# bennyguo/instant-nsr-pl

Measured on NVIDIA H100. Metric: rays/sec fwd+bwd (NeRF-Synthetic lego shape), higher is better.
Workload: dtype f16

## Files before the change

instant-nsr-pl_b200/csrc/nerf_fused_bwd.cu:

```cuda
#include <stdlib.h>
#include "nerf_fused.cuh"
#include "wgmma.cuh"

namespace {

constexpr int kWarps = 4;
constexpr int kThreads = kWarps * 32;
constexpr int kRows = kWarps * 16;
constexpr int kCtasPerSm = 2;

constexpr int T_X0 = 0;
constexpr int T_H1 = T_X0 + kRows * NF_LD32;
constexpr int T_CI = T_H1 + kRows * NSR_LD64;
constexpr int T_G1 = T_CI + kRows * NF_LD32;
constexpr int T_G2 = T_G1 + kRows * NSR_LD64;
constexpr int T_DC3 = T_G2 + kRows * NSR_LD64;
constexpr int T_DG2 = T_DC3 + kRows * 24;
constexpr int T_DG1 = T_DG2 + kRows * NSR_LD64;
constexpr int T_DO = T_DG1 + kRows * NSR_LD64;
constexpr int T_DH1 = T_DO + kRows * 24;
constexpr int T_X0B = T_DH1 + kRows * NSR_LD64;
constexpr int T_TOTAL = T_X0B + kRows * NF_LD32;
constexpr int S_XYZ = 0, S_DS = S_XYZ + kRows * 6, S_DRGB = S_DS + kRows, S_ROWF = S_DRGB + kRows * 3;
constexpr size_t kSmemBytes = (size_t)(NF_W_TOTAL + T_TOTAL) * sizeof(__half) + 2 * S_ROWF * sizeof(float);
// ... 499 lines not shown
            }
          }
        }
        a_dc3[0][0][0] = nsr_pack_h2(dp[0], dp[1]);
        a_dc3[0][0][1] = nsr_pack_h2(dp[2], dp[3]);
        a_dc3[0][0][2] = 0u;
        a_dc3[0][0][3] = 0u;
        canon_store_afrag<1>(a_dc3, slot + SL_DC3, 16, r0);
      }
      uint32_t a_d[1][4][4];
      nsr_zero_acc(acc);
      nsr_gemm_wt<1, 1, 8>(acc, a_dc3, W + NF_OFF_CW3, NSR_LD64);
      relu_mask_pack(acc, a_g2, a_d);
      canon_store_afrag<4>(a_d, slot + SL_DG2, 64, r0);
      nsr_zero_acc(acc);
      nsr_gemm_wt<1, 4, 8>(acc, a_d, W + NF_OFF_CW2, NSR_LD64);
      relu_mask_pack(acc, a_g1, a_d);
      canon_store_afrag<4>(a_d, slot + SL_DG1, 64, r0);
      nsr_zero_acc(acc16);
      nsr_gemm_wt<1, 4, 2>(acc16, a_d, W + NF_OFF_CW1, NF_LD32);
      if (c == 0) {
        if (ia < n) acc16[0][0][0] += dsr[0] * loss_scale;
        if (ib < n) acc16[0][0][2] += dsr[1] * loss_scale;
      }
      uint32_t a_do[1][1][4];
      nsr_acc_to_afrag<1, 2>(acc16, a_do, NSR_ACT_NONE);
      canon_store_afrag<1>(a_do, slot + SL_DO, 16, r0);
      nsr_zero_acc(acc);
      nsr_gemm_wt<1, 1, 8>(acc, a_do, W + NF_OFF_DW2, NSR_LD64);
      relu_mask_pack(acc, a_h1, a_d);
      canon_store_afrag<4>(a_d, slot + SL_DH1, 64, r0);
      nsr_proxy_fence();
      mbar_arrive(full_bar(s));
      float accE[1][4][4];
      nsr_zero_acc(accE);
      nsr_gemm_wt<1, 4, 4>(accE, a_d, W + NF_OFF_DW1, NF_LD32);
#pragma unroll
      for (int hh = 0; hh < 2; ++hh) {
        const int64_t i = hh ? ib : ia;
        if (i < n) {
#pragma unroll
          for (int nt = 0; nt < 4; ++nt) denc_out[i * 16 + nt * 4 + c] = nsr_pack_h2(accE[0][nt][hh * 2], accE[0][nt][hh * 2 + 1]);
        }
      }
    }
  } else {
    float w_dw1[16], w_dw2t[8], w_cw1[16], w_cw2[32], w_cw3t[8];
#pragma unroll
    for (int i = 0; i < 32; ++i) {
      if (i < 8) w_dw2t[i] = w_cw3t[i] = 0.f;
      if (i < 16) w_dw1[i] = w_cw1[i] = 0.f;
      w_cw2[i] = 0.f;
    }
    for (int64_t it = 0; it < my_tiles; ++it) {
      const int s = (int)(it % kNetSlots);
      mbar_wait(full_bar(s), (uint32_t)((it / kNetSlots) & 1), nullptr, 0);
      const uint32_t sl = sbase + N_SLOTS + (uint32_t)s * kSlotBytes;
      nsr_wg_fence();
#pragma unroll
      for (int kk = 0; kk < 4; ++kk) {
        nsr_wgmma_n32<1, 1>(w_dw1, nsr_wg_desc_mn(sl + SL_DH1, 64, kk), nsr_wg_desc_mn(sl + SL_X0, 32, kk), 1u);
        nsr_wgmma_n16<1, 1>(w_dw2t, nsr_wg_desc_mn(sl + SL_H1, 64, kk), nsr_wg_desc_mn(sl + SL_DO, 16, kk), 1u);
        nsr_wgmma_n32<1, 1>(w_cw1, nsr_wg_desc_mn(sl + SL_DG1, 64, kk), nsr_wg_desc_mn(sl + SL_CI, 32, kk), 1u);
        nsr_wgmma_n64<1, 1>(w_cw2, nsr_wg_desc_mn(sl + SL_DG2, 64, kk), nsr_wg_desc_mn(sl + SL_G1, 64, kk), 1u);
        nsr_wgmma_n16<1, 1>(w_cw3t, nsr_wg_desc_mn(sl + SL_G2, 64, kk), nsr_wg_desc_mn(sl + SL_DC3, 16, kk), 1u);
      }
      nsr_wg_commit();
      nsr_wg_wait0();
      nsr_wg_fence_regs(w_dw1);
      nsr_wg_fence_regs(w_dw2t);
      nsr_wg_fence_regs(w_cw1);
      nsr_wg_fence_regs(w_cw2);
      nsr_wg_fence_regs(w_cw3t);
      mbar_arrive(empty_bar(s));
    }
    if (my_tiles > 0) {
      net_flush(w_dw1, grad_dparams, 32, 1, inv_scale);
      net_flush(w_dw2t, grad_dparams + 64 * 32, 1, 64, inv_scale);
      net_flush(w_cw1, grad_cparams, 32, 1, inv_scale);
      net_flush(w_cw2, grad_cparams + 64 * 32, 64, 1, inv_scale);
      net_flush(w_cw3t, grad_cparams + 64 * 32 + 64 * 64, 1, 64, inv_scale);
    }
  }
}

}

namespace {

constexpr int kMergeLevels = 8;

template <int MINB>
__global__ void __launch_bounds__(256, MINB) nerf_table_scatter_kernel(const __grid_constant__ nsr_grid_t g, const float* __restrict__ xyz, int stride,
                                                                 const __half2* __restrict__ denc, float loss_scale,
                                                                 const float* __restrict__ amax_ptr, float* __restrict__ grad_table,
                                                                 int64_t n_cap, const int64_t* __restrict__ n_dev, int l_begin, int l_end) {
  const int64_t n = n_dev ? min(*n_dev, n_cap) : n_cap;
  if (loss_scale <= 0.f) {
    const float amax = fmaxf(__ldg(amax_ptr), 1e-30f);
    loss_scale = exp2f(fminf(fmaxf(floorf(log2f(256.f / amax)), -24.f), 60.f));
  }
  const float inv_scale = 1.f / loss_scale;
  const int lane = threadIdx.x & 31;
  const int64_t n32 = (n + 31) & ~31ll;
  for (int64_t i = blockIdx.x * 256ll + threadIdx.x; i < n32; i += (int64_t)gridDim.x * 256) {
    const bool ok = i < n;
    float x = 0.f, y = 0.f, z = 0.f;
    if (ok) {
      x = xyz[i * stride];
      y = xyz[i * stride + 1];
      z = xyz[i * stride + 2];
    }
    uint2 dq = make_uint2(0u, 0u);
#pragma unroll 1
    for (int l = l_begin; l < l_end; ++l) {
      float2 d = make_float2(0.f, 0.f);
      if (ok) {
        if (l == l_begin || (l & 1) == 0) dq = __ldg(reinterpret_cast<const uint2*>(denc + i * 16 + (l & ~1)));
        const uint32_t h = (l & 1) ? dq.y : dq.x;
        d = __half22float2(*reinterpret_cast<const __half2*>(&h));
        d.x *= inv_scale;
        d.y *= inv_scale;
      }
      const LevelInfo li = nsr_level(g, l);
      uint32_t cx, cy, cz, idx[8];
      float fx, fy, fz;
      nsr_pos_fract(x, li.scale, cx, fx);
      nsr_pos_fract(y, li.scale, cy, fy);
// ... 165 lines not shown
```

instant-nsr-pl_b200/fused.py:

```python
import ctypes
import math

import torch

from . import ops
from .lib import lib, ptr, stream, check_cuda, contig, NerfT
from .nerfacc import ContractionType

SCATTER_LEVEL_GROUPS = ((12, 16), (8, 12), (0, 8))


class _NerfRender(torch.autograd.Function):

    @staticmethod
    def forward(ctx, dparams, cparams, fused, rays, jitter):
        st = fused.trace(rays, jitter)
        n_rays, cap = rays.shape[0], st['cap']
        dev = rays.device
        acc_rgb = torch.zeros(n_rays, 3, device=dev)
        opacity = torch.zeros(n_rays, 1, device=dev)
        depth = torch.zeros(n_rays, 1, device=dev)
        sig = torch.empty(cap, device=dev)
        rgbs = torch.empty(cap, 3, device=dev)
        weights = torch.empty(cap, device=dev)
        need_grad = dparams.requires_grad or cparams.requires_grad
        enc = torch.empty(cap, 32, dtype=torch.float16, device=dev) if need_grad else None
        dh, ch = fused.dparams_half(), fused.cparams_half()
        k_dev = st['offsets_k'][n_rays:]
        lib.call('nsr_nerf_render_fwd', fused.ref(), ptr(rays), ptr(st['ri']), ptr(st['ts']), ptr(st['te']), ptr(st['trans']), ptr(dh),
                 ptr(ch), ptr(enc), ptr(sig), ptr(rgbs), ptr(weights), ptr(acc_rgb), ptr(opacity), ptr(depth), cap, ptr(k_dev), stream())
        ctx.fused, ctx.n_rays, ctx.cap = fused, n_rays, cap
        ctx.set_materialize_grads(False)
        ctx.save_for_backward(rays, st['ri'], st['ts'], st['te'], st['trans'], st['offsets_k'], enc, sig, rgbs, weights, dh, ch)
        counts = torch.cat([st['offsets_m'][n_rays:], k_dev])
        ctx.mark_non_differentiable(st['ri'], st['ts'], st['te'], counts)
        return acc_rgb, opacity, depth, weights, st['ri'], st['ts'], st['te'], counts

    @staticmethod
    def backward(ctx, g_rgb, g_op, g_depth, g_w, *_):
        fused = ctx.fused
        rays, ri, ts, te, trans, offsets_k, enc, sig, rgbs, weights, dh, ch = ctx.saved_tensors
        dev = rays.device
        n_rays, cap = ctx.n_rays, ctx.cap
        gd = torch.zeros(fused.n_dparams, device=dev)
        gc = torch.zeros(fused.n_cparams, device=dev)
        if cap > 0 and enc is not None:
            d_sraw = torch.empty(cap, device=dev)
            d_rgb = torch.empty(cap, 3, device=dev)
            amax = torch.zeros(1, device=dev)
            f32 = lambda t: None if t is None else contig(t, torch.float32)
            lib.call('nsr_nerf_ray_bwd', ptr(offsets_k), ptr(ts), ptr(te), ptr(trans), ptr(weights), ptr(sig), ptr(rgbs), ptr(f32(g_rgb)),
                     ptr(f32(g_op)), ptr(f32(g_depth)), ptr(f32(g_w)), ptr(d_sraw), ptr(d_rgb), ptr(amax), n_rays, stream())
            lib.call('nsr_nerf_field_bwd', fused.ref(), ptr(rays), ptr(ri), ptr(ts), ptr(te), ptr(enc), ptr(dh), ptr(ch), ptr(d_sraw),
                     ptr(d_rgb), ptr(gd), ptr(gc), float(fused.loss_scale), ptr(amax), cap, ptr(offsets_k[n_rays:]), None, None, stream())
        return gd, gc, None, None, None


class _NerfRenderRays(torch.autograd.Function):

    @staticmethod
    def forward(ctx, dparams, cparams, fused, rays, jitter):
        m = fused.model
# ... 53 lines not shown
        if packed_bwd:
            enc = None
        ctx.save_for_backward(rays, t_min, offsets_m, offsets_k, kept, enc, sig, rgbs, weights, trans, kidx, ri, ts, te, pos, dh, ch,
                              enc_k, xyzdir, amax0)
        ctx.mark_non_differentiable(ri, ts, te, pos, offsets_m, offsets_k, m_total, counts)
        return acc_rgb, opacity, depth, weights, ri, ts, te, pos, offsets_m, offsets_k, m_total, counts

    @staticmethod
    def backward(ctx, g_rgb, g_op, g_depth, g_w, *_):
        fused = ctx.fused
        rays, t_min, offsets_m, offsets_k, kept, enc, sig, rgbs, weights, trans, kidx, ri, ts, te, pos, dh, ch, enc_k, xyzdir, amax0 = ctx.saved_tensors
        dev = rays.device
        n, cap = ctx.n_rays, ctx.cap
        step = float(fused.model.render_step_size)
        direct = fused.direct_grads
        if direct is not None:
            gd, gc = direct
        else:
            gd = torch.empty(fused.n_dparams, device=dev)
            gc = torch.empty(fused.n_cparams, device=dev)
        n_head = fused.net.mlp.n_params
        split = fused.bwd_kernel == 'tiles_split' and enc_k is not None and n > 0
        (gd[:n_head] if split else gd).zero_()
        gc.zero_()
        if (enc is not None or enc_k is not None) and n > 0:
            f32 = lambda t: None if t is None else contig(t, torch.float32)
            amax = amax0
            if fused.bwd_kernel == 'rays':
                tick = torch.zeros(1, dtype=torch.int32, device=dev)
                lib.call('nsr_nerf_rays_bwd', fused.ref(), ptr(rays), ptr(t_min), ptr(offsets_m), ptr(kept), step, ptr(enc), ptr(sig), ptr(rgbs),
                         ptr(weights), ptr(trans), ptr(kidx), ptr(dh), ptr(ch), ptr(f32(g_rgb)), ptr(f32(g_op)), ptr(f32(g_depth)),
                         ptr(f32(g_w)), ptr(gd), ptr(gc), float(fused.loss_scale), ptr(amax), float(fused.t_bound), ptr(tick), n, stream())
            else:
                packed = enc_k is not None
                pad = 256 - cap % 128 if fused.bwd_kernel == 'tc' else 64
                d_sraw = torch.empty(cap + pad, device=dev)
                d_rgb = torch.empty(cap + pad, 3, device=dev)
                lib.call('nsr_nerf_ray_bwd_loose', ptr(offsets_m), ptr(kept), ptr(t_min), step, ptr(kidx), ptr(trans), ptr(weights), ptr(sig),
                         ptr(rgbs), ptr(f32(g_rgb)), ptr(f32(g_op)), ptr(f32(g_depth)), ptr(f32(g_w)), ptr(d_sraw), ptr(d_rgb), ptr(amax),
                         ptr(offsets_k) if packed else None, n, stream())
                if packed and fused.bwd_kernel == 'tc':
                    if fused._tc_status is None or fused._tc_status.device != dev:
                        fused._tc_status = torch.zeros(1, dtype=torch.int32, device=dev)
                    lib.call('nsr_nerf_field_bwd_tc', fused.ref(), ptr(enc_k), ptr(dh), ptr(ch), ptr(d_sraw), ptr(d_rgb), ptr(gd), ptr(gc),
                             float(fused.loss_scale), ptr(amax), cap, ptr(offsets_k[n:]), ptr(xyzdir), ptr(fused._tc_status), stream())
                elif packed and fused.bwd_kernel == 'tiles_split':
                    denc = torch.empty(cap, 32, dtype=torch.float16, device=dev)
                    lib.call('nsr_nerf_field_bwd_net', fused.ref(), ptr(enc_k), ptr(dh), ptr(ch), ptr(d_sraw), ptr(d_rgb), ptr(gd), ptr(gc),
                             float(fused.loss_scale), ptr(amax), cap, ptr(offsets_k[n:]), ptr(xyzdir), ptr(denc), stream())
                    groups = fused.level_groups or SCATTER_LEVEL_GROUPS
                    off = fused.grid.offset
                    if sorted(l for g in groups for l in range(*g)) != list(range(len(off) - 1)):
                        raise ValueError(f'level_groups {groups} must partition the {len(off) - 1} levels: the backward zeroes the table per group')
                    for gi, (l0, l1) in enumerate(groups):
                        gd[n_head + 2 * int(off[l0]):n_head + 2 * int(off[l1])].zero_()
                        lib.call('nsr_nerf_table_scatter', ctypes.byref(fused.struct.grid), ptr(xyzdir), 6, ptr(denc), float(fused.loss_scale), ptr(amax),
                                 ptr(gd[n_head:]), cap, ptr(offsets_k[n:]), l0, l1, 4 if (fused.exchange_hook is not None and gi > 0) else 0,
                                 stream())
                        if fused.exchange_hook is not None:
                            fused.exchange_hook(gi)
                else:
                    lib.call('nsr_nerf_field_bwd', fused.ref(), ptr(rays), ptr(ri), ptr(ts), ptr(te), ptr(enc_k if packed else enc), ptr(dh), ptr(ch),
                             ptr(d_sraw), ptr(d_rgb), ptr(gd), ptr(gc), float(fused.loss_scale), ptr(amax), cap, ptr(offsets_k[n:]),
                             None if packed else ptr(pos), ptr(xyzdir), stream())
        if direct is not None:
            return None, None, None, None, None
        return gd, gc, None, None, None


class NerfFused:

    def __init__(self, model):
        self.model = model
        geo, tex = model.geometry, model.texture
        self.net = geo.encoding_with_network
        self.cnet = tex.network
        self.grid = self.net.grid
        self.n_dparams, self.n_cparams = self.net.params.numel(), self.cnet.params.numel()
        r = float(model.config.radius)
        s = NerfT()
        s.grid = self.grid.struct
        s.radius = r
        s.density_bias = float(geo.config.density_bias)
        s.feature_dim, s.density_hidden, s.color_hidden = 16, 1, 2
        self.struct = s
        self.march = ops.march_struct([-r, -r, -r, r, r, r], model.occupancy_grid_res, ContractionType.AABB.value, model.render_step_size, 0.0)
        self.cap_per_ray = int(math.ceil(2.0 * math.sqrt(3.0) * r / model.render_step_size)) + 2
        self.loss_scale = 0.0
        self.early_stop_eps, self.alpha_thre = 1e-4, 0.0
        self.last_stats = {}
        self._ticket = None
        self.mode = 'per_ray'
        self.lean_static_outputs = False
        self.packed_bwd_inputs = True
        from .config import experimental
        self.fuse_kept_scan = experimental('pack_scan')
        import os
        self.bwd_kernel = os.environ.get('NSR_BWD_KERNEL', 'tiles_split')
        self._tc_status = None
        self.march_alloc = os.environ.get('NSR_MARCH_ALLOC', '1') == '1'
        self.direct_grads = None
        self._want_grad = True
        self.level_groups = None
        self.exchange_hook = None
        self.t_bound = 16.0

    @staticmethod
    def try_build(model):
        from . import tcnn
        from .models.fields import VolumeDensity, VolumeRadiance
        cfg = model.config
        geo, tex = model.geometry, model.texture
        try:
            ok = (not cfg.learned_background and cfg.grid_prune and isinstance(geo, VolumeDensity) and isinstance(tex, VolumeRadiance)
                  and isinstance(geo.encoding_with_network, tcnn.NetworkWithInputEncoding)
                  and geo.encoding_with_network.grid.n_levels == 16 and geo.encoding_with_network.mlp.n_hidden == 1
                  and geo.n_output_dims == 16 and geo.config.get('density_activation') == 'trunc_exp'
                  and 'feature_activation' not in geo.config
                  and isinstance(tex.network, tcnn.Network) and tex.network.mlp.n_hidden == 2 and tex.network.mlp.n_in == 32
                  and isinstance(tex.encoding.encoding, tcnn.Encoding) and tex.encoding.encoding.otype == 'SphericalHarmonics'
                  and not tex.encoding.include_xyz and tex.config.input_feature_dim == 16)
            dm, cm = geo.encoding_with_network.mlp.struct, tex.network.mlp.struct
            ok = ok and dm.activation == 1 and dm.out_activation == 0 and cm.activation == 1
            net_act = str(tex.network.network_config.get('output_activation', 'None')).lower()
            col_act = str(tex.config.get('color_activation', 'none')).lower()
            ok = ok and sorted([net_act, col_act]) == ['none', 'sigmoid']
        except AttributeError:
            ok = False
        return NerfFused(model) if ok else None

    def ref(self):
        return ctypes.byref(self.struct)

    def ticket(self, dev):
        if self._ticket is None or self._ticket.device != dev:
            self._ticket = torch.zeros(1, dtype=torch.int32, device=dev)
        return self._ticket

    def dparams_half(self):
        return self.net._params_half()

    def cparams_half(self):
        return self.cnet._params_half()

    @torch.no_grad()
    def density(self, positions):
        check_cuda(positions, what='NerfFused.density')
        p = contig(positions.reshape(-1, 3), torch.float32)
        out = torch.empty(p.shape[0], device=p.device)
        lib.call('nsr_nerf_density', self.ref(), ptr(p), ptr(self.dparams_half()), ptr(out), p.shape[0], stream())
        return out.reshape(positions.shape[:-1])

    @torch.no_grad()
    def trace(self, rays, jitter=None):
        m = self.model
        dev = rays.device
        n = rays.shape[0]
        cap = n * self.cap_per_ray
        mref = ctypes.byref(self.march)
        u = None
        if m.randomized:
            u = torch.rand(n, device=dev) if jitter is None else contig(jitter.to(dev), torch.float32)
        grid = m.occupancy_grid
        bits, coarse = grid.bits(), grid.coarse_bits()
        i32 = lambda k: torch.empty(k, dtype=torch.int32, device=dev)
        f32 = lambda k: torch.empty(k, dtype=torch.float32, device=dev)
        words = (self.cap_per_ray + 31) // 32
        masks, t_min = i32(n * words), f32(n)
        counts, offsets_m = i32(n), torch.empty(n + 1, dtype=torch.int64, device=dev)
        lib.call('nsr_march_rays_mask', mref, ptr(rays), ptr(u), ptr(bits), ptr(coarse), ptr(masks), words, ptr(t_min), ptr(counts), n, stream())
        lib.call('nsr_scan_counts', ptr(counts), ptr(offsets_m), n, stream())
        ri_m, ts_m, te_m = i32(cap), f32(cap), f32(cap)
        lib.call('nsr_march_rays_expand', mref, ptr(masks), words, ptr(t_min), ptr(offsets_m), ptr(ri_m), ptr(ts_m), ptr(te_m), n, stream())
        alphas = f32(cap)
        lib.call('nsr_nerf_prepass', self.ref(), ptr(rays), ptr(ri_m), ptr(ts_m), ptr(te_m), ptr(self.dparams_half()), ptr(alphas), cap,
                 ptr(offsets_m[n:]), stream())
        keep = torch.empty(cap, dtype=torch.uint8, device=dev)
        trans, kept = f32(cap), i32(n)
        lib.call('nsr_visibility', ptr(alphas), ptr(offsets_m), ptr(keep), ptr(trans), ptr(kept), self.early_stop_eps, self.alpha_thre, n, stream())
        offsets_k = torch.empty(n + 1, dtype=torch.int64, device=dev)
        lib.call('nsr_scan_counts', ptr(kept), ptr(offsets_k), n, stream())
        ri, ts, te, tr = i32(cap), f32(cap), f32(cap), f32(cap)
        lib.call('nsr_compact_prefix', ptr(offsets_m), ptr(offsets_k), ptr(ri_m), ptr(ts_m), ptr(te_m), ptr(trans), ptr(ri), ptr(ts), ptr(te),
                 ptr(tr), n, stream())
        return {'ri': ri, 'ts': ts, 'te': te, 'trans': tr, 'offsets_m': offsets_m, 'offsets_k': offsets_k, 'cap': cap}
# ... 54 lines not shown
```

instant-nsr-pl_b200/csrc/nerf_rays_fwd.cu:

```cuda
#include <stdlib.h>
#include "nerf_fused.cuh"

namespace {

constexpr int kWarps = 8;
constexpr int kThreads = kWarps * 32;
constexpr int kMaxWords = 64;
constexpr int kWarpHalves = 32 * NF_LD32 + 32 * 24 + 64 + 256;
constexpr size_t kSmemBytes = (size_t)(NF_W_TOTAL + kWarps * kWarpHalves) * sizeof(__half);

struct RaysFwdArgs {
  const float* rays;
  const uint32_t* masks;
  const float* t_min;
  const int64_t* offsets_m;
  const int32_t* order;
  const int32_t* bin_counts;
  const int32_t* counts;
  const __half* dparams;
  const __half* cparams;
  __half* enc_save;
  float* sigmas;
  float* rgbs;
  float* weights;
  float* trans;
  int32_t* kidx_out;
  float* acc_rgb;
  float* opacity;
  float* depth;
  int32_t* kept;
  int32_t* kept_blocks;
  uint32_t* ticket;
  float step, early_stop_eps;
  int words;
  int64_t n_rays;
};

__device__ __forceinline__ float warp_incl_prod(float v, int lane) {
#pragma unroll
  for (int o = 1; o < 32; o <<= 1) {
    const float t = __shfl_up_sync(0xffffffffu, v, o);
    if (lane >= o) v *= t;
  }
  return v;
}
__device__ __forceinline__ float warp_sum(float v) {
#pragma unroll
  for (int o = 16; o > 0; o >>= 1) v += __shfl_xor_sync(0xffffffffu, v, o);
  return v;
}

template <int MINB, int NB>
__global__ void __launch_bounds__(kThreads, MINB) nerf_rays_fwd_kernel(const __grid_constant__ nsr_nerf_t P, const RaysFwdArgs a) {
  extern __shared__ __align__(16) __half smem[];
  const int warp = threadIdx.x >> 5, lane = threadIdx.x & 31, g = lane >> 2, c = lane & 3;
  __half* At = smem + NF_W_TOTAL + warp * kWarpHalves;
  __half* St = At + 32 * NF_LD32;
  float* s_sig = reinterpret_cast<float*>(St + 32 * 24);
  float* s_rgb = s_sig + 32;
  const __half2* table = reinterpret_cast<const __half2*>(a.dparams + NF_DENSITY_PARAMS);
  nf_stage_weights(smem, a.dparams, a.cparams, true);
  __shared__ int bins[NSR_ORDER_BINS];
  if (threadIdx.x < NSR_ORDER_BINS) bins[threadIdx.x] = a.bin_counts != nullptr ? __ldg(a.bin_counts + threadIdx.x) : 0;
  __syncthreads();

  for (;;) {
    int64_t ray = 0;
    if (lane == 0) ray = atomicAdd(a.ticket, 1u);
    ray = __shfl_sync(0xffffffffu, ray, 0);
    if (ray >= a.n_rays) break;
    if (a.bin_counts != nullptr) {
      int t = (int)ray, b = 0;
#pragma unroll
      for (int q = 0; q < NSR_ORDER_BINS - 1; ++q) {
        const bool next = b == q && t >= bins[q];
        t -= next ? bins[q] : 0;
        b += next ? 1 : 0;
      }
      ray = __ldg(a.order + (int64_t)b * a.n_rays + t);
    } else if (a.order != nullptr) {
      ray = __ldg(a.order + ray);
    }
    const uint32_t mw0 = lane < a.words ? __ldg(a.masks + ray * a.words + lane) : 0u;
    const uint32_t mw1 = lane + 32 < a.words ? __ldg(a.masks + ray * a.words + lane + 32) : 0u;
    const int64_t base = a.offsets_m[ray];
    const int total = a.counts != nullptr ? __ldg(a.counts + ray) : (int)(a.offsets_m[ray + 1] - base);
    float o_acc = 0.f, d_acc = 0.f, r_acc = 0.f, g_acc = 0.f, b_acc = 0.f;
    int kept = 0;
    if (total > 0) {
      const float* rr = a.rays + ray * 6;
      const float ox = __ldg(rr + 0), oy = __ldg(rr + 1), oz = __ldg(rr + 2);
      const float dx = __ldg(rr + 3), dy = __ldg(rr + 4), dz = __ldg(rr + 5);
      const float tmin = __ldg(a.t_min + ray);
      const float inv = 1.f / (2.f * P.radius);
      float carry = 1.f;
      uint4 sh0, sh1;
      {
        float s[16];
        nsr_sh4(dx, dy, dz, s);
        sh0 = make_uint4(nsr_pack_h2(s[0], s[1]), nsr_pack_h2(s[2], s[3]), nsr_pack_h2(s[4], s[5]), nsr_pack_h2(s[6], s[7]));
        sh1 = make_uint4(nsr_pack_h2(s[8], s[9]), nsr_pack_h2(s[10], s[11]), nsr_pack_h2(s[12], s[13]), nsr_pack_h2(s[14], s[15]));
      }
      uint4* sp = reinterpret_cast<uint4*>(St + lane * 24);
      sp[0] = sh0;
      sp[1] = sh1;
      int cur_w = 0;
      uint32_t cur_m = __shfl_sync(0xffffffffu, mw0, 0);
      for (int b0 = 0; b0 < total; b0 += 32) {
        const int s_idx = b0 + lane;
        int k = -1, filled = 0;
        while (filled < 32) {
          if (cur_m == 0u) {
            if (++cur_w >= a.words) break;
            cur_m = cur_w < 32 ? __shfl_sync(0xffffffffu, mw0, cur_w) : __shfl_sync(0xffffffffu, mw1, cur_w - 32);
            continue;
          }
          const int cnt = __popc(cur_m), take = min(cnt, 32 - filled);
          if (lane >= filled && lane < filled + take) k = cur_w * 32 + (int)__fns(cur_m, 0, lane - filled + 1);
          if (take == cnt) {
            cur_m = 0u;
          } else {
            const uint32_t p = __fns(cur_m, 0, take);
            cur_m &= ~((2u << p) - 1u);
          }
          filled += take;
        }
        const bool valid = k >= 0;
        if (!valid) k = 0;
        const float t0 = __fmaf_rn((float)k, a.step, tmin), t1 = __fmaf_rn((float)k + 1.f, a.step, tmin);
        const float mid = (t0 + t1) * 0.5f;
        uint32_t f[16];
        if (valid) {
          const float x = (fmaf(dx, mid, ox) + P.radius) * inv, y = (fmaf(dy, mid, oy) + P.radius) * inv,
                      z = (fmaf(dz, mid, oz) + P.radius) * inv;
          nf_gather_batched<16, NB>(P.grid, table, x, y, z, f);
        } else {
#pragma unroll
          for (int l = 0; l < 16; ++l) f[l] = 0u;
        }
        nf_store_row32(At, lane, f);
        if (a.enc_save != nullptr && valid) {
          uint4* e = reinterpret_cast<uint4*>(a.enc_save + (base + s_idx) * 32);
          e[0] = make_uint4(f[0], f[1], f[2], f[3]);
          e[1] = make_uint4(f[4], f[5], f[6], f[7]);
          e[2] = make_uint4(f[8], f[9], f[10], f[11]);
          e[3] = make_uint4(f[12], f[13], f[14], f[15]);
        }
        __syncwarp();
        uint32_t a_o[2][1][4];
        {
          uint32_t a_in[2][2][4];
          nsr_load_afrag<2, 2>(a_in, At, NF_LD32, 0);
          float acc[2][8][4];
          nsr_zero_acc(acc);
          nsr_gemm_w<2, 2, 8>(acc, a_in, smem + NF_OFF_DW1, NF_LD32);
          uint32_t a_h[2][4][4];
          nsr_acc_to_afrag<2, 8>(acc, a_h, NSR_ACT_RELU);
          float acco[2][2][4];
          nsr_zero_acc(acco);
          nsr_gemm_w<2, 4, 2>(acco, a_h, smem + NF_OFF_DW2, NSR_LD64);
          nsr_acc_to_afrag<2, 2>(acco, a_o, NSR_ACT_NONE);
        }
        if (c == 0) {
#pragma unroll
          for (int m = 0; m < 2; ++m) {
            s_sig[m * 16 + g] = nf_half_lo(a_o[m][0][0]);
            s_sig[m * 16 + g + 8] = nf_half_lo(a_o[m][0][1]);
          }
        }
        {
          uint32_t a_c[2][2][4], a_sh[2][1][4];
          nsr_load_afrag<2, 1>(a_sh, St, 24, 0);
#pragma unroll
          for (int m = 0; m < 2; ++m)
#pragma unroll
            for (int j = 0; j < 4; ++j) {
              a_c[m][0][j] = a_o[m][0][j];
              a_c[m][1][j] = a_sh[m][0][j];
            }
          float acc[2][8][4];
          nsr_zero_acc(acc);
          nsr_gemm_w<2, 2, 8>(acc, a_c, smem + NF_OFF_CW1, NF_LD32);
          uint32_t a_h[2][4][4];
          nsr_acc_to_afrag<2, 8>(acc, a_h, NSR_ACT_RELU);
          nsr_zero_acc(acc);
          nsr_gemm_w<2, 4, 8>(acc, a_h, smem + NF_OFF_CW2, NSR_LD64);
          nsr_acc_to_afrag<2, 8>(acc, a_h, NSR_ACT_RELU);
          float acco[2][2][4];
          nsr_zero_acc(acco);
          nsr_gemm_w<2, 4, 2>(acco, a_h, smem + NF_OFF_CW3, NSR_LD64);
          uint32_t a_r[2][1][4];
          nsr_acc_to_afrag<2, 2>(acco, a_r, NSR_ACT_NONE);
          if (c < 2) {
#pragma unroll
            for (int m = 0; m < 2; ++m) {
              float* r0 = s_rgb + (m * 16 + g) * 4 + c * 2;
              float* r1 = s_rgb + (m * 16 + g + 8) * 4 + c * 2;
              r0[0] = nf_half_lo(a_r[m][0][0]);
              r0[1] = nf_half_hi(a_r[m][0][0]);
              r1[0] = nf_half_lo(a_r[m][0][1]);
              r1[1] = nf_half_hi(a_r[m][0][1]);
            }
          }
        }
        __syncwarp();
        const float sigma = expf(s_sig[lane] + P.density_bias);
        const float alpha = valid ? 1.f - expf(-sigma * (t1 - t0)) : 0.f;
        const float incl = warp_incl_prod(1.f - alpha, lane);
        float excl = __shfl_up_sync(0xffffffffu, incl, 1);
        if (lane == 0) excl = 1.f;
        const float T = carry * excl;
        const bool keep = valid && (T >= a.early_stop_eps);
        if (keep) {
          const float w = T * alpha;
          const float cr = 1.f / (1.f + expf(-s_rgb[lane * 4 + 0])), cg = 1.f / (1.f + expf(-s_rgb[lane * 4 + 1])),
                      cb = 1.f / (1.f + expf(-s_rgb[lane * 4 + 2]));
          o_acc += w;
          d_acc += w * mid;
          r_acc += w * cr;
          g_acc += w * cg;
          b_acc += w * cb;
          const int64_t p = base + s_idx;
          a.sigmas[p] = sigma;
          a.weights[p] = w;
          a.trans[p] = T;
          a.kidx_out[p] = k;
          a.rgbs[p * 3 + 0] = cr;
          a.rgbs[p * 3 + 1] = cg;
          a.rgbs[p * 3 + 2] = cb;
        }
        kept += __popc(__ballot_sync(0xffffffffu, keep));
        carry *= __shfl_sync(0xffffffffu, incl, 31);
        __syncwarp();
        if (carry < a.early_stop_eps) break;
      }
    }
    o_acc = warp_sum(o_acc);
    d_acc = warp_sum(d_acc);
    r_acc = warp_sum(r_acc);
    g_acc = warp_sum(g_acc);
    b_acc = warp_sum(b_acc);
    if (lane == 0) {
      a.opacity[ray] = o_acc;
      a.depth[ray] = d_acc;
      a.acc_rgb[ray * 3 + 0] = r_acc;
      a.acc_rgb[ray * 3 + 1] = g_acc;
      a.acc_rgb[ray * 3 + 2] = b_acc;
      a.kept[ray] = kept;
      if (a.kept_blocks != nullptr && kept > 0) atomicAdd(a.kept_blocks + (ray >> 8), kept);
    }
    __syncwarp();
  }
}

template <bool SCAN>
__global__ void __launch_bounds__(256) pack_kept_kernel(const int64_t* __restrict__ off_m, const int64_t* __restrict__ off_k,
                                                        const int32_t* __restrict__ kept, int64_t* __restrict__ off_k_out,
                                                        const float* __restrict__ t_min, float step, const int32_t* __restrict__ kidx,
                                                        const float* __restrict__ weights, int32_t* __restrict__ ri_k,
                                                        float* __restrict__ ts_k, float* __restrict__ te_k, float* __restrict__ w_k,
                                                        int64_t* __restrict__ loose_pos, const __grid_constant__ nsr_nerf_t P,
                                                        const float* __restrict__ rays, const uint4* __restrict__ enc_loose,
                                                        uint4* __restrict__ enc_k, float* __restrict__ xyzdir_k, int enc_tiled, int64_t n_rays,
                                                        const int32_t* __restrict__ kept_blocks) {
  const int lane = threadIdx.x & 31;
  const int64_t ray = blockIdx.x * 8ll + (threadIdx.x >> 5);
  int64_t dst, cnt;
  if (SCAN) {
    __shared__ int64_t s_part[8];
    const int64_t ray0 = blockIdx.x * 8ll;
    int64_t sum = 0;
    if (kept_blocks != nullptr) {
      const int64_t nb = ray0 >> 8;
      for (int64_t b = threadIdx.x; b < nb; b += 256) sum += __ldg(kept_blocks + b);
      for (int64_t r = (nb << 8) + threadIdx.x; r < ray0; r += 256) sum += __ldg(kept + r);
    } else {
      for (int64_t r = threadIdx.x; r < ray0; r += 256) sum += __ldg(kept + r);
    }
#pragma unroll
    for (int o = 16; o > 0; o >>= 1) sum += __shfl_xor_sync(0xffffffffu, sum, o);
    if (lane == 0) s_part[threadIdx.x >> 5] = sum;
    __syncthreads();
    int64_t base = 0;
#pragma unroll
    for (int w = 0; w < 8; ++w) base += s_part[w];
    for (int64_t r = ray0; r < ray && r < n_rays; ++r) base += __ldg(kept + r);
    if (ray >= n_rays) return;
    dst = base;
    cnt = __ldg(kept + ray);
    if (lane == 0) {
      off_k_out[ray] = dst;
      if (ray == n_rays - 1) off_k_out[n_rays] = dst + cnt;
    }
  } else {
    if (ray >= n_rays) return;
    dst = off_k[ray];
    cnt = off_k[ray + 1] - dst;
  }
  const int64_t src = off_m[ray];
  const float tmin = t_min[ray];
  for (int64_t j = lane; j < cnt; j += 32) {
    const float k = (float)kidx[src + j];
    const float t0 = __fmaf_rn(k, step, tmin), t1 = __fmaf_rn(k + 1.f, step, tmin);
    ri_k[dst + j] = (int32_t)ray;
    ts_k[dst + j] = t0;
    te_k[dst + j] = t1;
    if (w_k) w_k[dst + j] = weights[src + j];
    if (loose_pos) loose_pos[dst + j] = src + j;
    if (xyzdir_k) {
      float x, y, z, dx, dy, dz;
      nf_sample_position(P, rays, (int)ray, t0, t1, x, y, z, dx, dy, dz);
      float* o = xyzdir_k + (dst + j) * 6;
      o[0] = x; o[1] = y; o[2] = z; o[3] = dx; o[4] = dy; o[5] = dz;
    }
  }
  if (enc_k && !enc_tiled) {
    for (int64_t v = lane; v < cnt * 4; v += 32) enc_k[dst * 4 + v] = enc_loose[src * 4 + v];
  } else if (enc_k) {
    for (int64_t v = lane; v < cnt * 4; v += 32) {
      const int64_t R = dst + (v >> 2);
      const int kc = (int)(v & 3), r = (int)(R & 127);
      enc_k[(R >> 7) * 512 + ((r >> 3) * 4 + kc) * 8 + (r & 7)] = enc_loose[src * 4 + v];
    }
  }
}

__global__ void __launch_bounds__(256) ray_bwd_loose_kernel(const int64_t* __restrict__ off_m, const int32_t* __restrict__ kept,
                                                            const float* __restrict__ t_min, float step, const int32_t* __restrict__ kidx,
                                                            const float* __restrict__ trans, const float* __restrict__ weights,
                                                            const float* __restrict__ sigmas, const float* __restrict__ rgbs,
                                                            const float* __restrict__ g_rgb, const float* __restrict__ g_opacity,
                                                            const float* __restrict__ g_depth, const float* __restrict__ g_weights,
                                                            float* __restrict__ d_sraw, float* __restrict__ d_rgb, float* __restrict__ amax,
                                                            const int64_t* __restrict__ off_k, int64_t n_rays) {
  const int lane = threadIdx.x & 31;
  const int64_t ray = blockIdx.x * 8ll + (threadIdx.x >> 5);
  if (ray >= n_rays) return;
  const int64_t beg = off_m[ray];
  const int64_t out0 = off_k ? off_k[ray] : beg;
  const int n = kept[ray];
  if (n <= 0) return;
  const float tmin = t_min[ray];
  const float gr = g_rgb ? g_rgb[ray * 3 + 0] : 0.f, gg = g_rgb ? g_rgb[ray * 3 + 1] : 0.f, gb = g_rgb ? g_rgb[ray * 3 + 2] : 0.f;
  const float go = g_opacity ? g_opacity[ray] : 0.f, gd = g_depth ? g_depth[ray] : 0.f;
  float carry = 0.f, vmax = 0.f;
  for (int cb = ((n - 1) / 32) * 32; cb >= 0; cb -= 32) {
    const int j = cb + lane;
    const bool ok = j < n;
    const int64_t i = beg + j;
    float w = 0.f, gi = 0.f, delta = 0.f;
    if (ok) {
      w = weights[i];
      const float kf = (float)kidx[i];
      const float t0 = __fmaf_rn(kf, step, tmin), t1 = __fmaf_rn(kf + 1.f, step, tmin);
      delta = t1 - t0;
      gi = gr * rgbs[i * 3 + 0] + gg * rgbs[i * 3 + 1] + gb * rgbs[i * 3 + 2] + go + gd * ((t0 + t1) * 0.5f) + (g_weights ? g_weights[i] : 0.f);
      d_rgb[(out0 + j) * 3 + 0] = w * gr;
      d_rgb[(out0 + j) * 3 + 1] = w * gg;
      d_rgb[(out0 + j) * 3 + 2] = w * gb;
      vmax = fmaxf(vmax, 0.25f * w * fmaxf(fabsf(gr), fmaxf(fabsf(gg), fabsf(gb))));
    }
    const float gw = gi * w;
    float suf = gw;
#pragma unroll
    for (int o = 1; o < 32; o <<= 1) {
      const float t = __shfl_down_sync(0xffffffffu, suf, o);
      if (lane + o < 32) suf += t;
    }
    if (ok) {
      const float ds = delta * (gi * (trans[i] - w) - (carry + suf - gw));
      const float dr = ds * fminf(sigmas[i], 3269017.37f);
      d_sraw[out0 + j] = dr;
      vmax = fmaxf(vmax, fabsf(dr));
    }
    carry += __shfl_sync(0xffffffffu, suf, 0);
  }
  if (amax != nullptr) {
#pragma unroll
    for (int o = 16; o > 0; o >>= 1) vmax = fmaxf(vmax, __shfl_xor_sync(0xffffffffu, vmax, o));
    if (lane == 0 && vmax > 0.f && isfinite(vmax)) atomicMax(reinterpret_cast<int*>(amax), __float_as_int(vmax));
  }
}

}

extern "C" int nsr_nerf_rays_fwd(const nsr_nerf_t* f, const float* rays, const uint32_t* masks, int32_t words, const float* t_min,
                                 const int64_t* offsets_m, const int32_t* order, float step, float early_stop_eps, const void* dparams_h, const void* cparams_h,
                                 void* enc_save_h, float* sigmas, float* rgbs, float* weights, float* trans, int32_t* kidx,
                                 float* acc_rgb, float* opacity, float* depth, int32_t* kept, uint32_t* ticket, int64_t n_rays,
                                 const int32_t* counts, const int32_t* bin_counts, int32_t* kept_blocks, void* stream) {
  NSR_REQUIRE(bin_counts == nullptr || (order != nullptr && counts != nullptr), "nsr_nerf_rays_fwd: the binned queue needs order [8][n] and counts");
  NSR_REQUIRE(f != nullptr && f->grid.n_levels == 16 && f->grid.n_features == 2 && f->feature_dim == 16 && f->density_hidden == 1 &&
                  f->color_hidden == 2,
              "nsr_nerf_rays_fwd: fused path needs L=16, F=2, feature_dim=16, hidden layers 1/2");
  NSR_REQUIRE(words >= 1 && words <= kMaxWords, "nsr_nerf_rays_fwd: words must be in [1,%d]", kMaxWords);
  NSR_REQUIRE(ticket != nullptr && kept != nullptr, "nsr_nerf_rays_fwd: ticket / kept are required");
  if (n_rays == 0) return 0;
  static const int gather_batch = [] {
    const char* v = getenv("NSR_FWD_BATCH");
    return (v != nullptr && v[0] == '8') ? 8 : 4;
  }();
  static thread_local bool attr_set = false;
  if (!attr_set) {
    cudaError_t e = cudaFuncSetAttribute(nerf_rays_fwd_kernel<2, 4>, cudaFuncAttributeMaxDynamicSharedMemorySize, (int)kSmemBytes);
    if (e == cudaSuccess) e = cudaFuncSetAttribute(nerf_rays_fwd_kernel<2, 8>, cudaFuncAttributeMaxDynamicSharedMemorySize, (int)kSmemBytes);
    if (e != cudaSuccess) {
      nsr_set_error("nsr_nerf_rays_fwd: cannot reserve %zu B shared memory: %s", kSmemBytes, cudaGetErrorString(e));
      return 2;
    }
    attr_set = true;
  }
  RaysFwdArgs a;
  a.rays = rays; a.masks = masks; a.t_min = t_min; a.offsets_m = offsets_m; a.order = order; a.bin_counts = bin_counts; a.counts = counts; a.kept_blocks = kept_blocks;
  a.dparams = (const __half*)dparams_h; a.cparams = (const __half*)cparams_h; a.enc_save = (__half*)enc_save_h;
  a.sigmas = sigmas; a.rgbs = rgbs; a.weights = weights; a.trans = trans; a.kidx_out = kidx;
  a.acc_rgb = acc_rgb; a.opacity = opacity; a.depth = depth; a.kept = kept; a.ticket = ticket;
  a.step = step; a.early_stop_eps = early_stop_eps; a.words = words; a.n_rays = n_rays;
  const int64_t want = (n_rays + kWarps - 1) / kWarps;
  int grid = (int)min((int64_t)nsr_sm_count() * 2, want > 0 ? want : (int64_t)1);
  if (gather_batch == 8)
    nerf_rays_fwd_kernel<2, 8><<<grid, kThreads, kSmemBytes, (cudaStream_t)stream>>>(*f, a);
  else
    nerf_rays_fwd_kernel<2, 4><<<grid, kThreads, kSmemBytes, (cudaStream_t)stream>>>(*f, a);
  NSR_CHECK_LAUNCH("nsr_nerf_rays_fwd");
  return 0;
}

extern "C" int nsr_pack_kept(const int64_t* offsets_m, const int64_t* offsets_k, const float* t_min, float step, const int32_t* kidx,
                             const float* weights, int32_t* ray_indices_k, float* t_starts_k, float* t_ends_k, float* weights_k,
                             int64_t* loose_pos, const nsr_nerf_t* f, const float* rays, const void* enc_loose_h, void* enc_k_h,
                             float* xyzdir_k, int32_t enc_tiled, int64_t n_rays, void* stream) {
  if (n_rays == 0) return 0;
  NSR_REQUIRE(xyzdir_k == nullptr || (f != nullptr && rays != nullptr), "nsr_pack_kept: xyzdir_k needs the field descriptor and the rays");
  NSR_REQUIRE(enc_k_h == nullptr || enc_loose_h != nullptr, "nsr_pack_kept: enc_k needs the loose encoding buffer");
  nsr_nerf_t dummy;
  memset(&dummy, 0, sizeof(dummy));
  dummy.radius = 1.f;
  pack_kept_kernel<false><<<nsr_blocks(n_rays, 8), 256, 0, (cudaStream_t)stream>>>(offsets_m, offsets_k, nullptr, nullptr, t_min, step, kidx, weights,
                                                                                   ray_indices_k, t_starts_k, t_ends_k, weights_k, loose_pos,
                                                                                   f ? *f : dummy, rays, (const uint4*)enc_loose_h,
                                                                                   (uint4*)enc_k_h, xyzdir_k, enc_tiled, n_rays, nullptr);
  NSR_CHECK_LAUNCH("nsr_pack_kept");
  return 0;
}

extern "C" int nsr_pack_kept_scan(const int64_t* offsets_m, const int32_t* kept, int64_t* offsets_k_out, const float* t_min, float step,
                                  const int32_t* kidx, const float* weights, int32_t* ray_indices_k, float* t_starts_k, float* t_ends_k,
                                  float* weights_k, int64_t* loose_pos, const nsr_nerf_t* f, const float* rays, const void* enc_loose_h,
                                  void* enc_k_h, float* xyzdir_k, int32_t enc_tiled, int64_t n_rays, const int32_t* kept_blocks, void* stream) {
  NSR_REQUIRE(kept != nullptr && offsets_k_out != nullptr, "nsr_pack_kept_scan: kept / offsets_k_out is NULL");
  if (n_rays == 0) {
    cudaMemsetAsync(offsets_k_out, 0, sizeof(int64_t), (cudaStream_t)stream);
    return 0;
  }
  NSR_REQUIRE(xyzdir_k == nullptr || (f != nullptr && rays != nullptr), "nsr_pack_kept_scan: xyzdir_k needs the field descriptor and the rays");
  NSR_REQUIRE(enc_k_h == nullptr || enc_loose_h != nullptr, "nsr_pack_kept_scan: enc_k needs the loose encoding buffer");
  nsr_nerf_t dummy;
  memset(&dummy, 0, sizeof(dummy));
// ... 20 lines not shown
```

Baseline: 14.79 million.

## Run coarse-level table scatter on a side stream concurrently with fine levels

When no exchange hook is set, the coarsest level group (levels 0-8) of the hash-table gradient scatter is launched on a separate CUDA stream with a limited CTA-per-SM budget. The finer groups run on the main stream at the same time, and the main stream waits on the side stream afterwards. The aim is to overlap the small, contention-heavy coarse scatter with the larger fine-level scatters and fill otherwise idle SMs. This adds stream sync overhead and the two streams may compete for atomics bandwidth. A compile-time-gated clock64 probe in the net warpgroup is also added; it is off by default.

```diff
diff --git a/instant-nsr-pl_b200/csrc/nerf_fused_bwd.cu b/instant-nsr-pl_b200/csrc/nerf_fused_bwd.cu
--- a/instant-nsr-pl_b200/csrc/nerf_fused_bwd.cu
+++ b/instant-nsr-pl_b200/csrc/nerf_fused_bwd.cu
@@ -575,9 +575,19 @@
       if (i < 16) w_dw1[i] = w_cw1[i] = 0.f;
       w_cw2[i] = 0.f;
     }
+#ifdef NSR_NET_WG_IDLE
+    const long long t_start = clock64();
+    long long t_full = 0, t_mma = 0;
+#endif
     for (int64_t it = 0; it < my_tiles; ++it) {
       const int s = (int)(it % kNetSlots);
+#ifdef NSR_NET_WG_IDLE
+      long long t0 = clock64();
+#endif
       mbar_wait(full_bar(s), (uint32_t)((it / kNetSlots) & 1), nullptr, 0);
+#ifdef NSR_NET_WG_IDLE
+      t_full += clock64() - t0;
+#endif
       const uint32_t sl = sbase + N_SLOTS + (uint32_t)s * kSlotBytes;
       nsr_wg_fence();
 #pragma unroll
@@ -589,7 +599,13 @@
         nsr_wgmma_n16<1, 1>(w_cw3t, nsr_wg_desc_mn(sl + SL_G2, 64, kk), nsr_wg_desc_mn(sl + SL_DC3, 16, kk), 1u);
       }
       nsr_wg_commit();
+#ifdef NSR_NET_WG_IDLE
+      t0 = clock64();
+#endif
       nsr_wg_wait0();
+#ifdef NSR_NET_WG_IDLE
+      t_mma += clock64() - t0;
+#endif
       nsr_wg_fence_regs(w_dw1);
       nsr_wg_fence_regs(w_dw2t);
       nsr_wg_fence_regs(w_cw1);
@@ -597,6 +613,11 @@
       nsr_wg_fence_regs(w_cw3t);
       mbar_arrive(empty_bar(s));
     }
+#ifdef NSR_NET_WG_IDLE
+    if (threadIdx.x == 256)
+      printf("nerf_bwd_net_kernel warpgroup: cta %d tiles %lld full_wait %lld wgmma_wait %lld total %lld cycles\n", (int)blockIdx.x, (long long)my_tiles,
+             t_full, t_mma, clock64() - t_start);
+#endif
     if (my_tiles > 0) {
       net_flush(w_dw1, grad_dparams, 32, 1, inv_scale);
       net_flush(w_dw2t, grad_dparams + 64 * 32, 1, 64, inv_scale);
diff --git a/instant-nsr-pl_b200/fused.py b/instant-nsr-pl_b200/fused.py
--- a/instant-nsr-pl_b200/fused.py
+++ b/instant-nsr-pl_b200/fused.py
@@ -8,6 +8,8 @@
 from .nerfacc import ContractionType
 
 SCATTER_LEVEL_GROUPS = ((12, 16), (8, 12), (0, 8))
+COARSE_MERGE_LEVELS = 8
+COARSE_SIDE_CTAS_PER_SM = 3
 
 
 class _NerfRender(torch.autograd.Function):
@@ -167,13 +169,25 @@
                     off = fused.grid.offset
                     if sorted(l for g in groups for l in range(*g)) != list(range(len(off) - 1)):
                         raise ValueError(f'level_groups {groups} must partition the {len(off) - 1} levels: the backward zeroes the table per group')
-                    for gi, (l0, l1) in enumerate(groups):
+                    def scatter(l0, l1, ctas):
                         gd[n_head + 2 * int(off[l0]):n_head + 2 * int(off[l1])].zero_()
                         lib.call('nsr_nerf_table_scatter', ctypes.byref(fused.struct.grid), ptr(xyzdir), 6, ptr(denc), float(fused.loss_scale), ptr(amax),
-                                 ptr(gd[n_head:]), cap, ptr(offsets_k[n:]), l0, l1, 4 if (fused.exchange_hook is not None and gi > 0) else 0,
-                                 stream())
-                        if fused.exchange_hook is not None:
-                            fused.exchange_hook(gi)
+                                 ptr(gd[n_head:]), cap, ptr(offsets_k[n:]), l0, l1, ctas, stream())
+
+                    if fused.exchange_hook is None and len(groups) > 1 and groups[-1][1] <= COARSE_MERGE_LEVELS:
+                        main = torch.cuda.current_stream()
+                        side = fused.side_stream(dev)
+                        side.wait_stream(main)
+                        with torch.cuda.stream(side):
+                            scatter(*groups[-1], COARSE_SIDE_CTAS_PER_SM)
+                        for l0, l1 in groups[:-1]:
+                            scatter(l0, l1, 0)
+                        main.wait_stream(side)
+                    else:
+                        for gi, (l0, l1) in enumerate(groups):
+                            scatter(l0, l1, 4 if (fused.exchange_hook is not None and gi > 0) else 0)
+                            if fused.exchange_hook is not None:
+                                fused.exchange_hook(gi)
                 else:
                     lib.call('nsr_nerf_field_bwd', fused.ref(), ptr(rays), ptr(ri), ptr(ts), ptr(te), ptr(enc_k if packed else enc), ptr(dh), ptr(ch),
                              ptr(d_sraw), ptr(d_rgb), ptr(gd), ptr(gc), float(fused.loss_scale), ptr(amax), cap, ptr(offsets_k[n:]),
@@ -213,6 +227,7 @@
         import os
         self.bwd_kernel = os.environ.get('NSR_BWD_KERNEL', 'tiles_split')
         self._tc_status = None
+        self._side = None
         self.march_alloc = os.environ.get('NSR_MARCH_ALLOC', '1') == '1'
         self.direct_grads = None
         self._want_grad = True
@@ -246,6 +261,11 @@
 
     def ref(self):
         return ctypes.byref(self.struct)
+
+    def side_stream(self, dev):
+        if self._side is None or self._side.device != dev:
+            self._side = torch.cuda.Stream(device=dev)
+        return self._side
 
     def ticket(self, dev):
         if self._ticket is None or self._ticket.device != dev:
```

Result: faster. 15.09 million (median of 6 runs) (+2.0%).

## Keep SH and sigma in registers, shrink per-warp smem, batch compaction loads

Applied to the files above, without the earlier changes.

The fused NeRF forward kernel no longer stages spherical-harmonic features and raw sigma through shared memory. SH halves are built directly as MMA A-fragment registers, and sigma is gathered with warp shuffles, which cuts per-warp scratch and sets a shared-memory carveout sized for two CTAs. The compaction kernel now batches the kidx/weight loads and the uint4 encoding copies to raise memory-level parallelism. Risks are higher register pressure and a hard-coded 233472-byte divisor in the carveout calculation.

```diff
diff --git a/instant-nsr-pl_b200/csrc/nerf_rays_fwd.cu b/instant-nsr-pl_b200/csrc/nerf_rays_fwd.cu
--- a/instant-nsr-pl_b200/csrc/nerf_rays_fwd.cu
+++ b/instant-nsr-pl_b200/csrc/nerf_rays_fwd.cu
@@ -6,8 +6,9 @@
 constexpr int kWarps = 8;
 constexpr int kThreads = kWarps * 32;
 constexpr int kMaxWords = 64;
-constexpr int kWarpHalves = 32 * NF_LD32 + 32 * 24 + 64 + 256;
+constexpr int kWarpHalves = 32 * NF_LD32 + 256;
 constexpr size_t kSmemBytes = (size_t)(NF_W_TOTAL + kWarps * kWarpHalves) * sizeof(__half);
+static_assert(2 * (kSmemBytes + 1024) <= 100 * 1024, "two CTAs (+1 KB reserved each) must fit the 100 KB shared-memory configuration");
 
 struct RaysFwdArgs {
   const float* rays;
@@ -55,9 +56,7 @@
   extern __shared__ __align__(16) __half smem[];
   const int warp = threadIdx.x >> 5, lane = threadIdx.x & 31, g = lane >> 2, c = lane & 3;
   __half* At = smem + NF_W_TOTAL + warp * kWarpHalves;
-  __half* St = At + 32 * NF_LD32;
-  float* s_sig = reinterpret_cast<float*>(St + 32 * 24);
-  float* s_rgb = s_sig + 32;
+  float* s_rgb = reinterpret_cast<float*>(At + 32 * NF_LD32);
   const __half2* table = reinterpret_cast<const __half2*>(a.dparams + NF_DENSITY_PARAMS);
   nf_stage_weights(smem, a.dparams, a.cparams, true);
   __shared__ int bins[NSR_ORDER_BINS];
@@ -94,16 +93,15 @@
       const float tmin = __ldg(a.t_min + ray);
       const float inv = 1.f / (2.f * P.radius);
       float carry = 1.f;
-      uint4 sh0, sh1;
+      uint32_t sh_lo, sh_hi;
       {
         float s[16];
         nsr_sh4(dx, dy, dz, s);
-        sh0 = make_uint4(nsr_pack_h2(s[0], s[1]), nsr_pack_h2(s[2], s[3]), nsr_pack_h2(s[4], s[5]), nsr_pack_h2(s[6], s[7]));
-        sh1 = make_uint4(nsr_pack_h2(s[8], s[9]), nsr_pack_h2(s[10], s[11]), nsr_pack_h2(s[12], s[13]), nsr_pack_h2(s[14], s[15]));
+        const uint32_t p0 = nsr_pack_h2(s[0], s[1]), p1 = nsr_pack_h2(s[2], s[3]), p2 = nsr_pack_h2(s[4], s[5]), p3 = nsr_pack_h2(s[6], s[7]);
+        const uint32_t p4 = nsr_pack_h2(s[8], s[9]), p5 = nsr_pack_h2(s[10], s[11]), p6 = nsr_pack_h2(s[12], s[13]), p7 = nsr_pack_h2(s[14], s[15]);
+        sh_lo = c == 0 ? p0 : c == 1 ? p1 : c == 2 ? p2 : p3;
+        sh_hi = c == 0 ? p4 : c == 1 ? p5 : c == 2 ? p6 : p7;
       }
-      uint4* sp = reinterpret_cast<uint4*>(St + lane * 24);
-      sp[0] = sh0;
-      sp[1] = sh1;
       int cur_w = 0;
       uint32_t cur_m = __shfl_sync(0xffffffffu, mw0, 0);
       for (int b0 = 0; b0 < total; b0 += 32) {
@@ -161,23 +159,25 @@
           nsr_gemm_w<2, 4, 2>(acco, a_h, smem + NF_OFF_DW2, NSR_LD64);
           nsr_acc_to_afrag<2, 2>(acco, a_o, NSR_ACT_NONE);
         }
-        if (c == 0) {
+        float sig_raw;
+        {
+          const int src = (lane & 7) * 4;
+          const uint32_t v00 = __shfl_sync(0xffffffffu, a_o[0][0][0], src), v01 = __shfl_sync(0xffffffffu, a_o[0][0][1], src);
+          const uint32_t v10 = __shfl_sync(0xffffffffu, a_o[1][0][0], src), v11 = __shfl_sync(0xffffffffu, a_o[1][0][1], src);
+          const uint32_t v = lane < 8 ? v00 : lane < 16 ? v01 : lane < 24 ? v10 : v11;
+          sig_raw = nf_half_lo(v);
+        }
+        {
+          uint32_t a_c[2][2][4];
 #pragma unroll
           for (int m = 0; m < 2; ++m) {
-            s_sig[m * 16 + g] = nf_half_lo(a_o[m][0][0]);
-            s_sig[m * 16 + g + 8] = nf_half_lo(a_o[m][0][1]);
+#pragma unroll
+            for (int j = 0; j < 4; ++j) a_c[m][0][j] = a_o[m][0][j];
+            a_c[m][1][0] = sh_lo;
+            a_c[m][1][1] = sh_lo;
+            a_c[m][1][2] = sh_hi;
+            a_c[m][1][3] = sh_hi;
           }
-        }
-        {
-          uint32_t a_c[2][2][4], a_sh[2][1][4];
-          nsr_load_afrag<2, 1>(a_sh, St, 24, 0);
-#pragma unroll
-          for (int m = 0; m < 2; ++m)
-#pragma unroll
-            for (int j = 0; j < 4; ++j) {
-              a_c[m][0][j] = a_o[m][0][j];
-              a_c[m][1][j] = a_sh[m][0][j];
-            }
           float acc[2][8][4];
           nsr_zero_acc(acc);
           nsr_gemm_w<2, 2, 8>(acc, a_c, smem + NF_OFF_CW1, NF_LD32);
@@ -204,7 +204,7 @@
           }
         }
         __syncwarp();
-        const float sigma = expf(s_sig[lane] + P.density_bias);
+        const float sigma = expf(sig_raw + P.density_bias);
         const float alpha = valid ? 1.f - expf(-sigma * (t1 - t0)) : 0.f;
         const float incl = warp_incl_prod(1.f - alpha, lane);
         float excl = __shfl_up_sync(0xffffffffu, incl, 1);
@@ -299,28 +299,56 @@
   }
   const int64_t src = off_m[ray];
   const float tmin = t_min[ray];
-  for (int64_t j = lane; j < cnt; j += 32) {
-    const float k = (float)kidx[src + j];
-    const float t0 = __fmaf_rn(k, step, tmin), t1 = __fmaf_rn(k + 1.f, step, tmin);
-    ri_k[dst + j] = (int32_t)ray;
-    ts_k[dst + j] = t0;
-    te_k[dst + j] = t1;
-    if (w_k) w_k[dst + j] = weights[src + j];
-    if (loose_pos) loose_pos[dst + j] = src + j;
-    if (xyzdir_k) {
-      float x, y, z, dx, dy, dz;
-      nf_sample_position(P, rays, (int)ray, t0, t1, x, y, z, dx, dy, dz);
-      float* o = xyzdir_k + (dst + j) * 6;
-      o[0] = x; o[1] = y; o[2] = z; o[3] = dx; o[4] = dy; o[5] = dz;
-    }
-  }
-  if (enc_k && !enc_tiled) {
-    for (int64_t v = lane; v < cnt * 4; v += 32) enc_k[dst * 4 + v] = enc_loose[src * 4 + v];
-  } else if (enc_k) {
-    for (int64_t v = lane; v < cnt * 4; v += 32) {
-      const int64_t R = dst + (v >> 2);
-      const int kc = (int)(v & 3), r = (int)(R & 127);
-      enc_k[(R >> 7) * 512 + ((r >> 3) * 4 + kc) * 8 + (r & 7)] = enc_loose[src * 4 + v];
+  constexpr int kRowBatch = 4, kEncBatch = 8;
+  for (int64_t j0 = lane; j0 < cnt; j0 += 32 * kRowBatch) {
+    int32_t kb[kRowBatch];
+    float wb[kRowBatch];
+#pragma unroll
+    for (int u = 0; u < kRowBatch; ++u) {
+      const int64_t j = j0 + 32 * u;
+      kb[u] = j < cnt ? kidx[src + j] : 0;
+      wb[u] = j < cnt && w_k ? weights[src + j] : 0.f;
+    }
+#pragma unroll
+    for (int u = 0; u < kRowBatch; ++u) {
+      const int64_t j = j0 + 32 * u;
+      if (j >= cnt) break;
+      const float k = (float)kb[u];
+      const float t0 = __fmaf_rn(k, step, tmin), t1 = __fmaf_rn(k + 1.f, step, tmin);
+      ri_k[dst + j] = (int32_t)ray;
+      ts_k[dst + j] = t0;
+      te_k[dst + j] = t1;
+      if (w_k) w_k[dst + j] = wb[u];
+      if (loose_pos) loose_pos[dst + j] = src + j;
+      if (xyzdir_k) {
+        float x, y, z, dx, dy, dz;
+        nf_sample_position(P, rays, (int)ray, t0, t1, x, y, z, dx, dy, dz);
+        float* o = xyzdir_k + (dst + j) * 6;
+        o[0] = x; o[1] = y; o[2] = z; o[3] = dx; o[4] = dy; o[5] = dz;
+      }
+    }
+  }
+  if (enc_k) {
+    const int64_t n4 = cnt * 4;
+    for (int64_t v0 = lane; v0 < n4; v0 += 32 * kEncBatch) {
+      uint4 e[kEncBatch];
+#pragma unroll
+      for (int u = 0; u < kEncBatch; ++u) {
+        const int64_t v = v0 + 32 * u;
+        if (v < n4) e[u] = enc_loose[src * 4 + v];
+      }
+#pragma unroll
+      for (int u = 0; u < kEncBatch; ++u) {
+        const int64_t v = v0 + 32 * u;
+        if (v >= n4) break;
+        if (!enc_tiled) {
+          enc_k[dst * 4 + v] = e[u];
+        } else {
+          const int64_t R = dst + (v >> 2);
+          const int kc = (int)(v & 3), r = (int)(R & 127);
+          enc_k[(R >> 7) * 512 + ((r >> 3) * 4 + kc) * 8 + (r & 7)] = e[u];
+        }
+      }
     }
   }
 }
@@ -404,6 +432,9 @@
   if (!attr_set) {
     cudaError_t e = cudaFuncSetAttribute(nerf_rays_fwd_kernel<2, 4>, cudaFuncAttributeMaxDynamicSharedMemorySize, (int)kSmemBytes);
     if (e == cudaSuccess) e = cudaFuncSetAttribute(nerf_rays_fwd_kernel<2, 8>, cudaFuncAttributeMaxDynamicSharedMemorySize, (int)kSmemBytes);
+    const int carve = (int)((2 * (kSmemBytes + 1024) * 100 + 233471) / 233472);
+    if (e == cudaSuccess) e = cudaFuncSetAttribute(nerf_rays_fwd_kernel<2, 4>, cudaFuncAttributePreferredSharedMemoryCarveout, carve);
+    if (e == cudaSuccess) e = cudaFuncSetAttribute(nerf_rays_fwd_kernel<2, 8>, cudaFuncAttributePreferredSharedMemoryCarveout, carve);
     if (e != cudaSuccess) {
       nsr_set_error("nsr_nerf_rays_fwd: cannot reserve %zu B shared memory: %s", kSmemBytes, cudaGetErrorString(e));
       return 2;
```

Result: faster. 14.73 million before, 14.99 million after (median of 6 runs) (+1.7%).
